# haoningwu3639/StoryGen

Measured on AMD Instinct MI355X. Metric: UNet denoising steps/sec @512x512, 3 prior-frame ctx, bs=1, higher is better.
Workload: dtype f16; 1 GPU; BASELINE configs[1]: StoryGen denoising loop, 512x512 (64x64x4 latent), R=3 prior frames, CFG batch 3, DDIM, SD-1.5 UNet + attn3 (909M params, synthetic fp16 weights); stage=multi-image-condition, samples_per_gpu=1, parallelism=dp1 (one sample per GPU, final all-gather), hipgraph=True, dedup_identical_reference_samples=True, overlap_ref_pass_of_next_step=True, ref_ahead=1, warmup_run=5, split_graphs=False, stream_priority=False, ref_pass_on_cus=0, ref_pass_eager=False, paired_gemm_launches=True, paired_text_image_attention=False, groupnorm_stats_from_epilogues=True, fp16_block_stream=False

## Files before the change

### storygen_amd/csrc/attention.hip

```cpp
#include "attention_kernel.h"

using namespace sgattn;


static int attn_params(const sg_attn_desc* d, AttnParams& p, const char* who) {
    SG_REQUIRE(d != nullptr, "%s: null descriptor", who);
    SG_REQUIRE(d->q && d->k && d->vt && d->o, "%s: null q/k/vt/o", who);
    SG_REQUIRE(d->B > 0 && d->H > 0 && d->Nq > 0 && d->Nk > 0, "%s: bad shape", who);
    if (d->D != 40 && d->D != 80 && d->D != 160)
        return sg_set_error(SG_EUNSUP, "%s: head dim %d not in {40, 80, 160}", who, d->D);
    SG_REQUIRE(d->kv_batches >= 0 && d->kv_batches <= d->B, "%s: kv_batches must be in [0, B]", who);
    SG_REQUIRE(d->ldq % 8 == 0 && d->ldk % 8 == 0 && d->ldvt % 8 == 0 && d->ldo % 4 == 0, "%s: row strides", who);
    SG_REQUIRE(d->bsq % 8 == 0 && d->bsk % 8 == 0 && d->bsvt % 8 == 0 && d->bso % 4 == 0, "%s: batch strides", who);
    SG_REQUIRE(sg_aligned16(d->q) && sg_aligned16(d->k) && sg_aligned16(d->vt) && sg_aligned16(d->o), "%s: 16-byte alignment", who);
    const int64_t hd = (int64_t)d->H * d->D;
    SG_REQUIRE(d->ldq >= hd && d->ldk >= hd && d->ldo >= hd, "%s: token stride smaller than H*D", who);
    SG_REQUIRE(d->ldvt >= ((d->Nk + 7) & ~7), "%s: ldvt must cover Nk rounded up to 8 keys", who);
    SG_REQUIRE((int64_t)d->D * d->ldvt < (1ll << 31), "%s: VT head slab too large for 32-bit offsets", who);
    p = AttnParams{};
    p.q = reinterpret_cast<const f16*>(d->q); p.ldq = d->ldq; p.bsq = d->bsq;
    p.k = reinterpret_cast<const f16*>(d->k); p.ldk = d->ldk; p.bsk = d->bsk;
    p.vt = reinterpret_cast<const f16*>(d->vt); p.ldvt = d->ldvt; p.bsvt = d->bsvt;
    p.o = reinterpret_cast<f16*>(d->o); p.ldo = d->ldo; p.bso = d->bso;
    p.B = d->B; p.H = d->H; p.Nq = d->Nq; p.Nk = d->Nk;
    p.kv_batches = d->kv_batches > 0 ? d->kv_batches : d->B;
    p.scale_log2 = d->scale * 1.44269504088896340736f;
    if (d->kv2_batches > 0) {
        SG_REQUIRE(d->k2 && d->vt2 && d->Nk2 > 0 && d->kv2_batches <= p.kv_batches, "%s: kv2_batches needs k2, vt2, Nk2 and at most kv_batches rows", who);
        SG_REQUIRE(d->bsk2 % 8 == 0 && d->bsvt2 % 8 == 0 && sg_aligned16(d->k2) && sg_aligned16(d->vt2), "%s: k2 / vt2 strides and alignment", who);
        SG_REQUIRE(d->ldvt >= ((d->Nk2 + 7) & ~7), "%s: ldvt must cover Nk2 rounded up to 8 keys", who);
        p.k2 = reinterpret_cast<const f16*>(d->k2); p.bsk2 = d->bsk2;
        p.vt2 = reinterpret_cast<const f16*>(d->vt2); p.bsvt2 = d->bsvt2;
        p.Nk2 = d->Nk2; p.kv2 = d->kv2_batches;
    }
    return SG_OK;
}

static bool attn_big(const sg_attn_desc* d) { return (long)sg_cdiv(d->Nq, 128) * d->H * d->B >= 512; }

static int attn_fwd(const sg_attn_desc* d, float* lse2, sg_stream_t stream) {
    AttnParams p;
    if (int rc = attn_params(d, p, "sg_attn_fwd_f16")) return rc;
    hipStream_t st = (hipStream_t)stream;
    if (lse2) {
        p.lse2 = lse2;
        if (d->D == 40) launch_attn<40, 4, 3, 1, false, true>(p, st);
        else if (d->D == 80) launch_attn<80, 4, 3, 1, false, true>(p, st);
        else launch_attn<160, 4, 3, 1, false, true>(p, st);
        SG_CHECK_LAUNCH("sg_attn_fwd_lse_f16");
        return SG_OK;
    }
    const bool big = attn_big(d);
    const SgOptions& opt = sg_options();
    const int sub2 = opt.attn_sub2, prio = opt.attn_prio;
    if (d->D == 40) {
        if (big && sub2 && d->Nk >= 256) launch_attn<40, 4, 2, 2>(p, st);
        else if (big && prio) launch_attn<40, 4, 3, 1, true>(p, st);
        else if (big && opt.attn_d40_general) launch_attn<40, 4, 3, 1, false, false, false, true>(p, st);
        else if (big && opt.attn_lean) launch_attn<40, 4, 3, 1, false, false, true>(p, st);
        else if (big) launch_attn<40, 4, 3>(p, st);
        else launch_attn<40, 2, 2>(p, st);
    }
    else if (d->D == 80) {
        const int v80 = opt.attn_d80;
        if (v80 == 1 || (v80 == 0 && big)) launch_attn<80, 4, 3>(p, st);
        else if (v80 == 2) launch_attn<80, 2, 3>(p, st);
        else launch_attn<80, 2, 2>(p, st);
    }
    else {
        const int v160 = opt.attn_d160;
        if (v160 == 4 && d->Nq <= 256 && d->Nk > KVBLK && (long)sg_cdiv(d->Nq, 32) * d->H * d->B <= 256) launch_attn_ksplit<160, 4>(p, st);
        else if (v160 == 1) launch_attn<160, 2, 3>(p, st);
        else if (v160 == 2) launch_attn<160, 4, 2>(p, st);
        else if (v160 == 3 || v160 == 4) launch_attn<160, 4, 3>(p, st);
        else launch_attn<160, 2, 2>(p, st);
    }
    SG_CHECK_LAUNCH("sg_attn_fwd_f16");
    return SG_OK;
}

extern "C" int sg_attn_fwd_f16(const sg_attn_desc* d, sg_stream_t stream) { return attn_fwd(d, nullptr, stream); }

extern "C" int sg_attn_fwd_pair_f16(const sg_attn_desc* d0, const sg_attn_desc* d1, sg_stream_t stream) {
    AttnParams p0, p1;
    if (int rc = attn_params(d0, p0, "sg_attn_fwd_pair_f16[0]")) return rc;
    if (int rc = attn_params(d1, p1, "sg_attn_fwd_pair_f16[1]")) return rc;
    const SgOptions& opt = sg_options();
    const bool same = d0->D == d1->D && d0->B == d1->B && d0->H == d1->H && d0->Nq == d1->Nq;
    const bool defaults = !opt.attn_sub2 && !opt.attn_prio && opt.attn_d80 == 1 && opt.attn_d160 >= 3;
    if (!same || !defaults) {
        if (int rc = attn_fwd(d0, nullptr, stream)) return rc;
        return attn_fwd(d1, nullptr, stream);
    }
    const AttnParams& a = p0.Nk >= p1.Nk ? p0 : p1;
    const AttnParams& b = p0.Nk >= p1.Nk ? p1 : p0;
    hipStream_t st = (hipStream_t)stream;
    if (d0->D == 40) {
        if (attn_big(d0)) launch_attn_pair<40, 4, 3>(a, b, st);
        else launch_attn_pair<40, 2, 2>(a, b, st);
    } else if (d0->D == 80) launch_attn_pair<80, 4, 3>(a, b, st);
    else launch_attn_pair<160, 4, 3>(a, b, st);
    SG_CHECK_LAUNCH("sg_attn_fwd_pair_f16");
    return SG_OK;
}

extern "C" int sg_attn_fwd_lse_f16(const sg_attn_desc* d, float* lse2, sg_stream_t stream) {
    SG_REQUIRE(lse2 != nullptr, "sg_attn_fwd_lse_f16: null lse2");
    return attn_fwd(d, lse2, stream);
}
```

### storygen_amd/csrc/attention_kernel.h

```cpp
#pragma once
#include "common.h"
#include <stdlib.h>

namespace sgattn {


constexpr int KVBLK = 64;
constexpr float RESCALE_THR = 6.0f;

struct AttnParams {
    const f16* q; long ldq, bsq;
    const f16* k; long ldk, bsk;
    const f16* vt; long ldvt, bsvt;
    f16* o; long ldo, bso;
    int B, H, Nq, Nk, kv_batches, nqb;
    const f16* k2; long bsk2; const f16* vt2; long bsvt2; int Nk2, kv2;
    float scale_log2;
    float* lse2;
};

__device__ __forceinline__ void glds16(const f16* g, char* lds_wave_base) {
    __builtin_amdgcn_global_load_lds((const __attribute__((address_space(1))) void*)g,
                                     (__attribute__((address_space(3))) void*)lds_wave_base, 16, 0, 0);
}
template <int N>
__device__ __forceinline__ void wait_vmcnt() {
    asm volatile("s_waitcnt vmcnt(%0)" ::"n"(N) : "memory");
}

template <int D>
__device__ __forceinline__ int kswz(int row) {
    return D == 40 ? 0 : (D == 80 ? ((row >> 3) & 1) : ((row >> 2) & 3));
}

constexpr int F40_KPAD = 2688;
constexpr int F40_ONES = 128;

template <int D, int S, int SUB>
constexpr int attn_smem_bytes() {
    return D == 40 ? F40_KPAD + S * SUB * (KVBLK * D * 2 + D * 128 + F40_ONES) : S * SUB * (KVBLK * D * 2 + D * 128) + (D % 16 == 0 ? 0 : 16);
}

#ifdef SG_ATTN_RT_STAGE
constexpr bool UNROLL_STAGES = false;
#else
constexpr bool UNROLL_STAGES = true;
#endif

template <int D, int NW, int S, int SUB, bool PRIO, bool LSE, bool LEAN = false, bool GENERAL = false, bool KSPLIT = false>
__device__ __forceinline__ void attn_fwd_body(const AttnParams& p, char* smem, const int block, const int nblocks) {
    constexpr bool F40 = D == 40 && !GENERAL;
    constexpr int DC = D / 8;
    constexpr int NDK = (D + 15) / 16;
    constexpr int DT = (D + 31) / 32;
    constexpr int KROW = D * 2;
    constexpr int K_BYTES = KVBLK * KROW;
    constexpr int V_BYTES = D * 128;
    constexpr int K_SEG = K_BYTES / 1024, V_SEG = V_BYTES / 1024, NSEG = K_SEG + V_SEG;
    constexpr int TSTAGE = K_BYTES + V_BYTES + (F40 ? F40_ONES : 0);
    constexpr int STAGE = SUB * TSTAGE;
    constexpr int RING0 = F40 ? F40_KPAD : 0;
    constexpr int MAXL = (NSEG + NW - 1) / NW;
    constexpr int REM = NSEG % NW;
    static_assert(KSPLIT ? (S == 1 && SUB == NW && !LSE && !(D == 40 && !GENERAL)) : (S == 2 || S == 3), "2 or 3 stages; key split: one stage of NW tiles");
    static_assert(KSPLIT || SUB == 1 || S == 2, "multi-tile stages use the 2-stage ring (plain vmcnt(0) waits)");
    static_assert(!KSPLIT || NW * (8 + DT * 64) * 64 <= S * SUB * (KVBLK * D * 2 + D * 128), "the merge images of the waves fit the dead ring");
    static_assert((S - 1) * MAXL < 64, "vmcnt is a 6-bit counter");
    static_assert(RING0 + S * STAGE + (F40 || D % 16 == 0 ? 0 : 16) <= attn_smem_bytes<D, S, SUB>(), "LDS size");
    static_assert(!F40 || (32 * KROW + 16 <= F40_KPAD && F40_KPAD % 128 == 0), "K pad constants of both 32-key blocks");

    const int t = threadIdx.x, lane = t & 63, l31 = lane & 31, hi = lane >> 5;
    const int wave = __builtin_amdgcn_readfirstlane(t >> 6);
    const int work = xcd_remap(block, nblocks);
    const int bh = work / p.nqb, qb = work - bh * p.nqb;
    const int h = bh / p.B, b = bh - h * p.B;
    const int kvb = b < p.kv_batches ? b : b - (p.B - p.kv_batches);
    const bool short_row = kvb < p.kv2;
    const int Nk = short_row ? p.Nk2 : p.Nk;
    const int q0 = KSPLIT ? qb * 32 : (qb * NW + wave) * 32;
    const f16* Q = p.q + (long)b * p.bsq + (long)h * D;
    const f16* K = (short_row ? p.k2 + (long)kvb * p.bsk2 : p.k + (long)(kvb - p.kv2) * p.bsk) + (long)h * D;
    const f16* VT = (short_row ? p.vt2 + (long)kvb * p.bsvt2 : p.vt + (long)(kvb - p.kv2) * p.bsvt) + (long)h * D * p.ldvt;
    const int nkp8 = (Nk + 7) & ~7;

    if constexpr (F40) {
// ... 274 lines not shown
            f16x8 vn[VPRE ? 1 : DT];
            if constexpr (!VPRE) {
                if (ks + 1 < 4) {
#pragma unroll
                    for (int i = 0; i < DT; ++i) {
                        const int d = min(i * 32 + l31, DLAST);
                        vn[i] = *reinterpret_cast<const f16x8*>(sV + d * 128 + ((((ks + 1) * 2 + hi) ^ ((d >> 1) & 7)) << 4));
                    }
                }
                __builtin_amdgcn_sched_barrier(0);
            }
            if constexpr (PRIO) __builtin_amdgcn_s_setprio(1);
#pragma unroll
            for (int i = 0; i < DT; ++i)
                oacc[i] = __builtin_amdgcn_mfma_f32_32x32x16_f16(vf[VPRE ? ks : 0][i], pf, oacc[i], 0, 0, 0);
            if constexpr (PRIO) __builtin_amdgcn_s_setprio(0);
            if constexpr (!VPRE) {
                if (ks + 1 < 4) {
#pragma unroll
                    for (int i = 0; i < DT; ++i) vf[0][i] = vn[i];
                }
            }
        }
        }
      }
        }
        if (!UNR && ++rt_stage == S) rt_stage = 0;
    }
    }

    float l_tot;
    if constexpr (F40) l_tot = oacc[DT - 1][4];
    else l_tot = l_run + __shfl_xor(l_run, 32, 64);
    if constexpr (KSPLIT) {
        constexpr int IMG = (8 + DT * 64) * 64;
        __builtin_amdgcn_s_barrier();
        if (wave > 0) {
            float* img = reinterpret_cast<float*>(smem + (wave - 1) * IMG);
            img[lane] = m_run;
            img[64 + lane] = l_tot;
#pragma unroll
            for (int i = 0; i < DT; ++i)
#pragma unroll
                for (int r = 0; r < 16; ++r) img[128 + (i * 16 + r) * 64 + lane] = oacc[i][r];
        }
        asm volatile("s_waitcnt lgkmcnt(0)" ::: "memory");
        __builtin_amdgcn_s_barrier();
        if (wave > 0) return;
#pragma unroll
        for (int w = 1; w < NW; ++w) {
            const float* img = reinterpret_cast<const float*>(smem + (w - 1) * IMG);
            const float m_o = img[lane], l_o = img[64 + lane];
            const float m_new = fmaxf(m_run, m_o);
            const float fa = __builtin_amdgcn_exp2f(m_run - m_new), fb = __builtin_amdgcn_exp2f(m_o - m_new);
            l_tot = l_tot * fa + l_o * fb;
            m_run = m_new;
#pragma unroll
            for (int i = 0; i < DT; ++i)
#pragma unroll
                for (int r = 0; r < 16; ++r) oacc[i][r] = oacc[i][r] * fa + img[128 + (i * 16 + r) * 64 + lane] * fb;
        }
    }
    const float inv = 1.0f / l_tot;
    const int qi = q0 + l31;
    if constexpr (LSE) {
        if (hi == 0 && qi < p.Nq) p.lse2[((long)b * p.H + h) * p.Nq + qi] = m_run + __log2f(l_tot);
    }
    if (qi < p.Nq) {
        f16* O = p.o + (long)b * p.bso + (long)qi * p.ldo + (long)h * D;
#pragma unroll
        for (int i = 0; i < DT; ++i)
#pragma unroll
            for (int g = 0; g < 4; ++g) {
                const int d0 = i * 32 + 8 * g + 4 * hi;
                if (d0 < D) {
                    f16x4 w = {(f16)(oacc[i][4 * g + 0] * inv), (f16)(oacc[i][4 * g + 1] * inv),
                               (f16)(oacc[i][4 * g + 2] * inv), (f16)(oacc[i][4 * g + 3] * inv)};
                    *reinterpret_cast<f16x4*>(O + d0) = w;
                }
            }
    }
}

template <int D, int NW, int S, int SUB = 1, bool PRIO = false, bool LSE = false, bool LEAN = false, bool GENERAL = false>
__global__ __launch_bounds__(64 * NW) void attn_fwd_kernel(const AttnParams p) {
    __shared__ __attribute__((aligned(16))) char smem[attn_smem_bytes<D, S, SUB>()];
    attn_fwd_body<D, NW, S, SUB, PRIO, LSE, LEAN, GENERAL>(p, smem, (int)blockIdx.x, (int)gridDim.x);
}

template <int D, int NW>
__global__ __launch_bounds__(64 * NW) void attn_fwd_ksplit_kernel(const AttnParams p) {
    __shared__ __attribute__((aligned(16))) char smem[attn_smem_bytes<D, 1, NW>()];
    attn_fwd_body<D, NW, 1, NW, false, false, false, false, true>(p, smem, (int)blockIdx.x, (int)gridDim.x);
}

template <int D, int NW>
void launch_attn_ksplit(const AttnParams& p0, hipStream_t st) {
    AttnParams p = p0;
    p.nqb = sg_cdiv(p.Nq, 32);
    hipLaunchKernelGGL((attn_fwd_ksplit_kernel<D, NW>), dim3(p.nqb * p.H * p.B), dim3(64 * NW), 0, st, p);
}

template <int D, int NW, int S>
__global__ __launch_bounds__(64 * NW) void attn_fwd_pair_kernel(const AttnParams a, const AttnParams b, const int na) {
    __shared__ __attribute__((aligned(16))) char smem[attn_smem_bytes<D, S, 1>()];
    if ((int)blockIdx.x < na) attn_fwd_body<D, NW, S, 1, false, false>(a, smem, (int)blockIdx.x, na);
    else attn_fwd_body<D, NW, S, 1, false, false>(b, smem, (int)blockIdx.x - na, (int)gridDim.x - na);
}

template <int D, int NW, int S, int SUB = 1, bool PRIO = false, bool LSE = false, bool LEAN = false, bool GENERAL = false>
void launch_attn(const AttnParams& p0, hipStream_t st) {
    AttnParams p = p0;
    p.nqb = sg_cdiv(p.Nq, 32 * NW);
    hipLaunchKernelGGL((attn_fwd_kernel<D, NW, S, SUB, PRIO, LSE, LEAN, GENERAL>), dim3(p.nqb * p.H * p.B), dim3(64 * NW), 0, st, p);
}

template <int D, int NW, int S>
void launch_attn_pair(const AttnParams& a0, const AttnParams& b0, hipStream_t st) {
    AttnParams a = a0, b = b0;
    a.nqb = sg_cdiv(a.Nq, 32 * NW); b.nqb = sg_cdiv(b.Nq, 32 * NW);
    const int na = a.nqb * a.H * a.B, nb = b.nqb * b.H * b.B;
    hipLaunchKernelGGL((attn_fwd_pair_kernel<D, NW, S>), dim3(na + nb), dim3(64 * NW), 0, st, a, b, na);
}


}
```

### storygen_amd/csrc/common.h

```cpp
#pragma once
#include <hip/hip_runtime.h>
#include <stdint.h>
#include <stdio.h>
#include <stdarg.h>

#include "../../include/storygen_hip.h"

typedef _Float16 f16;
typedef f16 f16x2 __attribute__((ext_vector_type(2)));
typedef f16 f16x4 __attribute__((ext_vector_type(4)));
typedef f16 f16x8 __attribute__((ext_vector_type(8)));
typedef float f32x4 __attribute__((ext_vector_type(4)));
typedef float f32x16 __attribute__((ext_vector_type(16)));

int sg_set_error(int code, const char* fmt, ...);

#define SG_REQUIRE(cond, ...)                                   \
    do {                                                        \
        if (!(cond)) return sg_set_error(SG_EINVAL, __VA_ARGS__); \
    } while (0)

#define SG_CHECK_LAUNCH(name)                                                                  \
    do {                                                                                       \
        hipError_t e__ = hipGetLastError();                                                    \
        if (e__ != hipSuccess) return sg_set_error(SG_ELAUNCH, "%s: %s", name, hipGetErrorString(e__)); \
    } while (0)

static inline bool sg_aligned16(const void* p) { return (reinterpret_cast<uintptr_t>(p) & 15u) == 0; }
static inline int sg_cdiv(long a, long b) { return (int)((a + b - 1) / b); }

struct SgOptions {
    int tile_m = 0, tile_n = 0;
    int no_pipe = 0, no_split = 0;
    int no_nmajor = 0;
    int pipe_stages = 3;
    int lat_tiles = 640;
    int lat_min_kt = 8, lat_max_kt = 64;
    int lat_stages = 4;
    int lat_mask = 62;
    int big_m = 0, big_bm = 0, big_bn = 0;
    int fat_m = 0;
    int lat_wide = 0, lat_wide_m = 256;
    int attn_sub2 = 0, attn_prio = 0, attn_d80 = 1, attn_d160 = 4 , attn_lean = 0;
    int attn_d40_general = 0;
    int gn_no_fused = 0, gn_wide = 1;
    int gn_fused_nt = 1024;
    int gn_chunks = 0;
    int ff_variant = 3;
    long gn_fused_max = -1;
};
SgOptions& sg_options();

__device__ __forceinline__ uint4 ldg16(const void* p) { return *reinterpret_cast<const uint4*>(p); }
__device__ __forceinline__ void stg16(void* p, uint4 v) { *reinterpret_cast<uint4*>(p) = v; }

union H8 {
    uint4 u;
    f16x8 v;
    f16 h[8];
};

__device__ __forceinline__ void load8f(const void* base, long off, bool f32, float (&v)[8]) {
    if (f32) {
        const float* q = reinterpret_cast<const float*>(base) + off;
        const float4 a = *reinterpret_cast<const float4*>(q), b = *reinterpret_cast<const float4*>(q + 4);
        v[0] = a.x; v[1] = a.y; v[2] = a.z; v[3] = a.w; v[4] = b.x; v[5] = b.y; v[6] = b.z; v[7] = b.w;
    } else {
        H8 h; h.u = ldg16(reinterpret_cast<const f16*>(base) + off);
#pragma unroll
        for (int j = 0; j < 8; ++j) v[j] = (float)h.h[j];
    }
}
__device__ __forceinline__ void store8h(f16* p, const float (&v)[8]) {
    H8 o;
#pragma unroll
    for (int j = 0; j < 8; ++j) o.h[j] = (f16)v[j];
    stg16(p, o.u);
}

__device__ __forceinline__ float silu_f(float x) { return x / (1.0f + __expf(-x)); }
__device__ __forceinline__ float gelu_erf_f(float x) {
    const float ax = fabsf(x);
    const float t = __builtin_amdgcn_rcpf(fmaf(ax, 0.3275911f * 0.70710678118654752440f, 1.0f));
    const float zs = ax * 0.84932180028801904272f;
    const float e = __builtin_amdgcn_exp2f(-zs * zs);
    float q = fmaf(1.061405429f, t, -1.453152027f);
    q = fmaf(q, t, 1.421413741f);
    q = fmaf(q, t, -0.284496736f);
    q = fmaf(q, t, 0.254829592f);
    q *= t;
    return 0.5f * fmaf(ax, fmaf(-q, e, 1.0f), x);
}

__device__ __forceinline__ float wave_sum(float v) {
#pragma unroll
    for (int o = 32; o > 0; o >>= 1) v += __shfl_xor(v, o, 64);
    return v;
}

__device__ __forceinline__ int xcd_remap(int bid, int nblocks) {
    const int q = nblocks >> 3, r = nblocks & 7;
    const int xcd = bid & 7, local = bid >> 3;
    const int base = (xcd < r) ? xcd * (q + 1) : r * (q + 1) + (xcd - r) * q;
    return base + local;
}
```

### storygen_amd/csrc/misc.hip

```cpp
#include "common.h"
#include <string.h>

static thread_local char g_err[512] = "";

SgOptions& sg_options() {
    static SgOptions o;
    return o;
}

extern "C" int sg_debug_set_option(const char* name, int64_t value) {
    if (!name) return sg_set_error(SG_EINVAL, "sg_debug_set_option: null name");
    SgOptions& o = sg_options();
    struct Entry { const char* n; int* p; };
    const Entry table[] = {{"tile_m", &o.tile_m}, {"tile_n", &o.tile_n}, {"no_pipe", &o.no_pipe}, {"no_split", &o.no_split},
                           {"no_nmajor", &o.no_nmajor}, {"attn_sub2", &o.attn_sub2}, {"attn_prio", &o.attn_prio},
                           {"attn_d80", &o.attn_d80}, {"attn_d160", &o.attn_d160}, {"gn_no_fused", &o.gn_no_fused},
                           {"gn_wide", &o.gn_wide}, {"attn_lean", &o.attn_lean}, {"attn_d40_general", &o.attn_d40_general},
                           {"gn_fused_nt", &o.gn_fused_nt}, {"pipe_stages", &o.pipe_stages}, {"ff_variant", &o.ff_variant},
                           {"gn_chunks", &o.gn_chunks}, {"lat_tiles", &o.lat_tiles}, {"lat_min_kt", &o.lat_min_kt},
                           {"lat_max_kt", &o.lat_max_kt}, {"lat_stages", &o.lat_stages}, {"lat_wide", &o.lat_wide}, {"lat_mask", &o.lat_mask}, {"lat_wide_m", &o.lat_wide_m}, {"fat_m", &o.fat_m}, {"big_m", &o.big_m}, {"big_bm", &o.big_bm}, {"big_bn", &o.big_bn}};
    for (const Entry& e : table)
        if (strcmp(e.n, name) == 0) {
            *e.p = (int)value;
            return SG_OK;
        }
    if (strcmp(name, "gn_fused_max") == 0) {
        o.gn_fused_max = (long)value;
        return SG_OK;
    }
    if (strcmp(name, "reset") == 0) {
        o = SgOptions{};
        return SG_OK;
    }
    return sg_set_error(SG_EINVAL, "sg_debug_set_option: unknown option '%s'", name);
}

int sg_set_error(int code, const char* fmt, ...) {
    va_list ap;
    va_start(ap, fmt);
    vsnprintf(g_err, sizeof(g_err), fmt, ap);
    va_end(ap);
    return code;
}

extern "C" int sg_version(void) { return 1; }
extern "C" const char* sg_last_error(void) { return g_err; }

extern "C" int sg_device_arch(void) {
    int dev = 0;
    hipDeviceProp_t prop;
    if (hipGetDevice(&dev) != hipSuccess || hipGetDeviceProperties(&prop, dev) != hipSuccess)
        return sg_set_error(SG_ELAUNCH, "sg_device_arch: no HIP device");
    const char* name = prop.gcnArchName;
    if (strncmp(name, "gfx", 3) != 0) return sg_set_error(SG_EARCH, "sg_device_arch: unexpected arch '%s'", name);
    return (int)strtol(name + 3, nullptr, 10);
}

extern "C" int sg_device_cus(void) {
    int dev = 0;
    hipDeviceProp_t prop;
    if (hipGetDevice(&dev) != hipSuccess || hipGetDeviceProperties(&prop, dev) != hipSuccess)
        return sg_set_error(SG_ELAUNCH, "sg_device_cus: no HIP device");
    return prop.multiProcessorCount;
}

namespace {

__global__ void timestep_embed_kernel(const float* t, const float* freqs, float* out, int B, int dim, int flip) {
    const int half = dim / 2;
    const int idx = blockIdx.x * blockDim.x + threadIdx.x;
    if (idx >= B * half) return;
    const int b = idx / half, j = idx - b * half;
    const float e = t[b] * freqs[j];
    const float s = sinf(e), c = cosf(e);
    float* o = out + (long)b * dim;
    if (flip) { o[j] = c; o[half + j] = s; } else { o[j] = s; o[half + j] = c; }
}

template <int MAXB>
__global__ __launch_bounds__(256) void linear_rows_kernel(const float* x, long ldx, const f16* W, long ldw, const f16* bias,
                                                          float* y, long ldy, int B, int N, int K, int act_in, int act_out) {
    const int lane = threadIdx.x & 63, n = blockIdx.x * 4 + (threadIdx.x >> 6);
    if (n >= N) return;
    float acc[MAXB];
#pragma unroll
    for (int b = 0; b < MAXB; ++b) acc[b] = 0.f;
    const f16* wr = W + (long)n * ldw;
    for (int k0 = lane * 8; k0 < K; k0 += 64 * 8) {
        H8 w; w.u = ldg16(wr + k0);
#pragma unroll
        for (int b = 0; b < MAXB; ++b) {
            if (b < B) {
                const float4 x0 = *reinterpret_cast<const float4*>(x + b * ldx + k0);
                const float4 x1 = *reinterpret_cast<const float4*>(x + b * ldx + k0 + 4);
                float xv[8] = {x0.x, x0.y, x0.z, x0.w, x1.x, x1.y, x1.z, x1.w};
#pragma unroll
                for (int j = 0; j < 8; ++j) {
                    const float a = act_in ? silu_f(xv[j]) : xv[j];
                    acc[b] += a * (float)w.h[j];
                }
// ... 337 lines not shown
```

### storygen_amd/ops.py

```python
from __future__ import annotations

import ctypes as C
from typing import Optional

import torch

from . import _lib
from ._lib import AttnDesc, ConvDesc, FfDesc, GemmDesc, GroupNormDesc, check

lib = _lib.load()

EPI_LINEAR = 0
EPI_GEGLU = 1
F_OUT_F32, F_RES1_F32, F_RES2_F32 = 1, 2, 4

TILE_TABLE = {}
TUNE_SINK = None


def _apply_tile(d, tile, split_k, sig, mn):
    if tile is not None:
        d.tile_m, d.tile_n = tile[0], tile[1]
        if len(tile) > 2:
            d.tile_waves = tile[2]
# ... 878 lines not shown
    d = AttnDesc()
    d.q, d.ldq, d.bsq = q.data_ptr(), q.stride(1), q.stride(0)
    d.k, d.ldk, d.bsk = k.data_ptr(), k.stride(1), k.stride(0)
    d.vt, d.ldvt, d.bsvt = vt.data_ptr(), vt.stride(1), vt.stride(0)
    d.o, d.ldo, d.bso = out.data_ptr(), out.stride(1), out.stride(0)
    d.B, d.H, d.Nq, d.Nk, d.D, d.kv_batches, d.scale = B, heads, Nq, Nk, D, (0 if Bk == B else Bk), scale
    return d


def attention_lse(q: torch.Tensor, k: torch.Tensor, vt: torch.Tensor, out: torch.Tensor, lse2: torch.Tensor, heads: int,
                  scale: float, nk: Optional[int] = None) -> torch.Tensor:
    _f32(lse2, "lse2")
    if tuple(lse2.shape) != (q.shape[0], heads, q.shape[1]) or not lse2.is_contiguous():
        raise ValueError("attention_lse: lse2 must be a contiguous [B, H, Nq]")
    d = _attn_desc(q, k, vt, out, heads, scale, nk)
    with _timed(f"attention_d{d.D}", 4.0 * d.B * d.H * d.Nq * d.Nk * d.D, f"B{d.B} H{d.H} Nq{d.Nq} Nk{d.Nk} lse"):
        check(lib.sg_attn_fwd_lse_f16(C.byref(d), lse2.data_ptr(), _stream()), "sg_attn_fwd_lse_f16")
    return out


def attention_bwd_prep(o: torch.Tensor, dout: torch.Tensor, lse2: torch.Tensor, ld2: torch.Tensor, heads: int) -> torch.Tensor:
    _f16(o, "o"), _f16(dout, "dout"), _f32(lse2, "lse2"), _f32(ld2, "ld2")
    B, Nq, Cq = o.shape
    if tuple(ld2.shape) != (B, heads, Nq, 2) or not ld2.is_contiguous() or not lse2.is_contiguous():
        raise ValueError("attention_bwd_prep: ld2 must be a contiguous [B, H, Nq, 2], lse2 a contiguous [B, H, Nq]")
    check(lib.sg_attn_bwd_prep_f32(o.data_ptr(), o.stride(1), o.stride(0), dout.data_ptr(), dout.stride(1), dout.stride(0),
                                   lse2.data_ptr(), ld2.data_ptr(), B, heads, Nq, Cq // heads, _stream()), "sg_attn_bwd_prep_f32")
    return ld2


def _attn_bwd_desc(q, k, v, dout, ld2, heads, scale):
    from ._lib import AttnBwdDesc
    for n, t in (("q", q), ("k", k), ("v", v), ("dout", dout)):
        _f16(t, n)
        if t.dim() != 3 or t.stride(2) != 1:
            raise ValueError(f"attention_bwd: {n} must be [B, N, H*D] with a contiguous last dimension")
    _f32(ld2, "ld2")
    B, Nq, Cq = q.shape
    d = AttnBwdDesc()
    d.q, d.ldq, d.bsq = q.data_ptr(), q.stride(1), q.stride(0)
    d.k, d.ldk, d.bsk = k.data_ptr(), k.stride(1), k.stride(0)
    d.v, d.ldv, d.bsv = v.data_ptr(), v.stride(1), v.stride(0)
    d.dout, d.lddo, d.bsdo = dout.data_ptr(), dout.stride(1), dout.stride(0)
    d.ld2 = ld2.data_ptr()
    d.B, d.H, d.Nq, d.Nk, d.D, d.scale = B, heads, Nq, k.shape[1], Cq // heads, scale
    return d


def attention_bwd_dq(q: torch.Tensor, k: torch.Tensor, kt: torch.Tensor, v: torch.Tensor, dout: torch.Tensor, ld2: torch.Tensor,
                     dq: torch.Tensor, heads: int, scale: float) -> torch.Tensor:
    d = _attn_bwd_desc(q, k, v, dout, ld2, heads, scale)
    _f16(kt, "kt"), _f16(dq, "dq")
    d.kt, d.ldkt, d.bskt = kt.data_ptr(), kt.stride(1), kt.stride(0)
    d.dq, d.lddq, d.bsdq = dq.data_ptr(), dq.stride(1), dq.stride(0)
    with _timed("attention_bwd", 6.0 * d.B * d.H * d.Nq * d.Nk * d.D, f"dq B{d.B} H{d.H} Nq{d.Nq} Nk{d.Nk} D{d.D}"):
        check(lib.sg_attn_bwd_dq_f16(C.byref(d), _stream()), "sg_attn_bwd_dq_f16")
    return dq


def attention_bwd_dkv(q: torch.Tensor, qt: torch.Tensor, k: torch.Tensor, v: torch.Tensor, dout: torch.Tensor, dot: torch.Tensor,
                      ld2: torch.Tensor, dkt: torch.Tensor, dvt: torch.Tensor, heads: int, scale: float):
    d = _attn_bwd_desc(q, k, v, dout, ld2, heads, scale)
    for n, t in (("qt", qt), ("dot", dot), ("dkt", dkt), ("dvt", dvt)):
        _f16(t, n)
    d.qt, d.ldqt, d.bsqt = qt.data_ptr(), qt.stride(1), qt.stride(0)
    d.dot, d.lddot, d.bsdot = dot.data_ptr(), dot.stride(1), dot.stride(0)
    d.dkt, d.lddkt, d.bsdkt = dkt.data_ptr(), dkt.stride(1), dkt.stride(0)
    d.dvt, d.lddvt, d.bsdvt = dvt.data_ptr(), dvt.stride(1), dvt.stride(0)
    with _timed("attention_bwd", 8.0 * d.B * d.H * d.Nq * d.Nk * d.D, f"dkv B{d.B} H{d.H} Nq{d.Nq} Nk{d.Nk} D{d.D}"):
        check(lib.sg_attn_bwd_dkv_f16(C.byref(d), _stream()), "sg_attn_bwd_dkv_f16")
    return dkt, dvt


def debug_set_tile(bm: int = 0, bn: int = 0, no_pipe: bool = False) -> None:
    check(lib.sg_debug_set_tile(bm, bn, int(no_pipe)), "sg_debug_set_tile")


def debug_set_option(name: str, value: int) -> None:
    check(lib.sg_debug_set_option(name.encode(), int(value)), "sg_debug_set_option")


_ENV_OPTIONS = {"SG_NO_NMAJOR": "no_nmajor", "SG_NO_PIPE": "no_pipe", "SG_NO_SPLIT": "no_split",
                "SG_ATTN_SUB2": "attn_sub2", "SG_ATTN_PRIO": "attn_prio", "SG_ATTN_D80": "attn_d80", "SG_ATTN_D160": "attn_d160",
                "SG_FF_VARIANT": "ff_variant", "SG_PIPE_STAGES": "pipe_stages", "SG_GN_FUSED_NT": "gn_fused_nt", "SG_GN_CHUNKS": "gn_chunks", "SG_ATTN_LEAN": "attn_lean", "SG_ATTN_D40_GENERAL": "attn_d40_general", "SG_NO_GN_FUSED": "gn_no_fused", "SG_GN_WIDE": "gn_wide", "SG_GN_FUSED_MAX": "gn_fused_max",
                "SG_LAT_TILES": "lat_tiles", "SG_LAT_MIN_KT": "lat_min_kt", "SG_LAT_MAX_KT": "lat_max_kt", "SG_LAT_STAGES": "lat_stages", "SG_LAT_WIDE": "lat_wide", "SG_LAT_MASK": "lat_mask", "SG_LAT_WIDE_M": "lat_wide_m", "SG_FAT_M": "fat_m", "SG_BIG_M": "big_m", "SG_BIG_BM": "big_bm", "SG_BIG_BN": "big_bn"}


def apply_env_options() -> dict:
    import os
    done = {}
    for var, name in _ENV_OPTIONS.items():
        if os.environ.get(var, "") != "":
            debug_set_option(name, int(os.environ[var]))
            done[name] = int(os.environ[var])
    if os.environ.get("SG_TILE"):
        bm, bn = (int(v) for v in os.environ["SG_TILE"].split(","))
        debug_set_option("tile_m", bm), debug_set_option("tile_n", bn)
        done["tile"] = (bm, bn)
    return done


def debug_mfma_f8(a_bytes: torch.Tensor, b_bytes: torch.Tensor, scale_a: int = 127, scale_b: int = 127) -> torch.Tensor:
    if a_bytes.dtype != torch.uint8 or tuple(a_bytes.shape) != (64, 32) or not a_bytes.is_cuda or not a_bytes.is_contiguous():
        raise TypeError("debug_mfma_f8: a must be a contiguous CUDA uint8 [64, 32]")
    if b_bytes.dtype != torch.uint8 or tuple(b_bytes.shape) != (64, 32) or not b_bytes.is_cuda or not b_bytes.is_contiguous():
        raise TypeError("debug_mfma_f8: b must be a contiguous CUDA uint8 [64, 32]")
    out = torch.empty(64, 16, dtype=torch.float32, device=a_bytes.device)
    check(lib.sg_debug_mfma_f8_32x32x64(a_bytes.data_ptr(), b_bytes.data_ptr(), out.data_ptr(), scale_a, scale_b, _stream()),
          "sg_debug_mfma_f8_32x32x64")
    return out


def debug_mfma(a: torch.Tensor, b: torch.Tensor) -> torch.Tensor:
    out = torch.empty(64, 16, dtype=torch.float32, device=a.device)
    check(lib.sg_debug_mfma_32x32x16(a.data_ptr(), b.data_ptr(), out.data_ptr(), _stream()), "sg_debug_mfma_32x32x16")
    return out
```

Measured before the change: 78.03 denoising steps/s.

## Add specialized head-dim-40 attention kernel with precomputed load offsets and compile-time stages

Adds a dedicated D=40 flash-attention kernel and makes it the default for single and paired launches; the old generic path stays behind an option. It precomputes per-wave global-to-LDS offsets and splits the K/V^T load segments across waves, with waves 0 and 1 loading the extra segment. The main loop is unrolled over compile-time ring stages, and full tiles skip masking. It also folds the running max into the Q fragment so the MFMA subtracts it, and sets waves_per_eu(3). The aim is to cut address arithmetic, branching and masking overhead in the D=40 attention at 64x64 resolution, at the cost of a large new specialized code path that carries precision and correctness risk.

```diff
diff --git a/storygen_amd/csrc/attention.hip b/storygen_amd/csrc/attention.hip
--- a/storygen_amd/csrc/attention.hip
+++ b/storygen_amd/csrc/attention.hip
@@ -58,8 +58,9 @@
         else if (big && prio) launch_attn<40, 4, 3, 1, true>(p, st);
         else if (big && opt.attn_d40_general) launch_attn<40, 4, 3, 1, false, false, false, true>(p, st);
         else if (big && opt.attn_lean) launch_attn<40, 4, 3, 1, false, false, true>(p, st);
-        else if (big) launch_attn<40, 4, 3>(p, st);
-        else launch_attn<40, 2, 2>(p, st);
+        else if (opt.attn_d40_loop == 1) big ? launch_attn<40, 4, 3>(p, st) : launch_attn<40, 2, 2>(p, st);
+        else if (big) launch_attn_d40<4, 3>(p, st);
+        else launch_attn_d40<2, 2>(p, st);
     }
     else if (d->D == 80) {
         const int v80 = opt.attn_d80;
@@ -87,7 +88,8 @@
     if (int rc = attn_params(d1, p1, "sg_attn_fwd_pair_f16[1]")) return rc;
     const SgOptions& opt = sg_options();
     const bool same = d0->D == d1->D && d0->B == d1->B && d0->H == d1->H && d0->Nq == d1->Nq;
-    const bool defaults = !opt.attn_sub2 && !opt.attn_prio && opt.attn_d80 == 1 && opt.attn_d160 >= 3;
+    const bool defaults = !opt.attn_sub2 && !opt.attn_prio && opt.attn_d80 == 1 && opt.attn_d160 >= 3 &&
+                          !(d0->D == 40 && opt.attn_d40_loop == 1);
     if (!same || !defaults) {
         if (int rc = attn_fwd(d0, nullptr, stream)) return rc;
         return attn_fwd(d1, nullptr, stream);
@@ -96,8 +98,8 @@
     const AttnParams& b = p0.Nk >= p1.Nk ? p1 : p0;
     hipStream_t st = (hipStream_t)stream;
     if (d0->D == 40) {
-        if (attn_big(d0)) launch_attn_pair<40, 4, 3>(a, b, st);
-        else launch_attn_pair<40, 2, 2>(a, b, st);
+        if (attn_big(d0)) launch_attn_d40_pair<4, 3>(a, b, st);
+        else launch_attn_d40_pair<2, 2>(a, b, st);
     } else if (d0->D == 80) launch_attn_pair<80, 4, 3>(a, b, st);
     else launch_attn_pair<160, 4, 3>(a, b, st);
     SG_CHECK_LAUNCH("sg_attn_fwd_pair_f16");
diff --git a/storygen_amd/csrc/attention_kernel.h b/storygen_amd/csrc/attention_kernel.h
--- a/storygen_amd/csrc/attention_kernel.h
+++ b/storygen_amd/csrc/attention_kernel.h
@@ -1,6 +1,7 @@
 #pragma once
 #include "common.h"
 #include <stdlib.h>
+#include <type_traits>
 
 namespace sgattn {
 
@@ -441,6 +442,312 @@
     }
 }
 
+template <int NW, int S>
+__device__ __forceinline__ void attn_d40_body(const AttnParams& p, char* smem, const int block, const int nblocks) {
+    constexpr int D = 40, DC = D / 8, NDK = 3, DT = 2, KROW = D * 2;
+    constexpr int K_BYTES = KVBLK * KROW, V_BYTES = D * 128;
+    constexpr int K_SEG = K_BYTES / 1024, V_SEG = V_BYTES / 1024;
+    constexpr int TSTAGE = K_BYTES + V_BYTES + F40_ONES, RING0 = F40_KPAD;
+    constexpr int NPAIR = (K_SEG - 1) / NW;
+    static_assert((NW == 2 || NW == 4) && (S == 2 || S == 3), "2 or 4 waves, 2 or 3 stages");
+    static_assert(K_SEG == 5 && V_SEG == 5 && NPAIR * NW == 4, "4 segments of K and of V^T over the waves + one of each for waves 0 and 1");
+    static_assert(RING0 + S * TSTAGE <= attn_smem_bytes<D, S, 1>(), "LDS size");
+
+    const int t = threadIdx.x, lane = t & 63, l31 = lane & 31, hi = lane >> 5;
+    const int wave = __builtin_amdgcn_readfirstlane(t >> 6);
+    const int work = xcd_remap(block, nblocks);
+    const int bh = work / p.nqb, qb = work - bh * p.nqb;
+    const int h = bh / p.B, b = bh - h * p.B;
+    const int kvb = b < p.kv_batches ? b : b - (p.B - p.kv_batches);
+    const bool short_row = kvb < p.kv2;
+    const int Nk = short_row ? p.Nk2 : p.Nk;
+    const int q0 = (qb * NW + wave) * 32;
+    const f16* Q = p.q + (long)b * p.bsq + (long)h * D;
+    const f16* K = (short_row ? p.k2 + (long)kvb * p.bsk2 : p.k + (long)(kvb - p.kv2) * p.bsk) + (long)h * D;
+    const f16* VT = (short_row ? p.vt2 + (long)kvb * p.bsvt2 : p.vt + (long)(kvb - p.kv2) * p.bsvt) + (long)h * D * p.ldvt;
+    const int nkp8 = (Nk + 7) & ~7;
+    const int ntiles = (Nk + KVBLK - 1) / KVBLK, nfull = Nk / KVBLK;
+    const int ldk = (int)p.ldk, ldvt = (int)p.ldvt;
+
+    if (t < 8) {
+        const unsigned v = (t & 3) == 0 ? 0x3C003C00u : 0u;
+        *reinterpret_cast<unsigned*>(smem + ((t >> 2) ? 32 * KROW : 0) + 4 * (t & 3)) = v;
+    }
+    for (int i = t; i < S * (F40_ONES / 4); i += 64 * NW) {
+        const int img = i / (F40_ONES / 4), w = i - img * (F40_ONES / 4);
+        *reinterpret_cast<unsigned*>(smem + RING0 + img * TSTAGE + K_BYTES + V_BYTES + 4 * w) = 0x3C003C00u;
+    }
+    asm volatile("s_waitcnt lgkmcnt(0)" ::: "memory");
+
+    auto kcoord = [&](int seg, int& row, int& col) __attribute__((always_inline)) {
+        const int s = seg * 64 + lane;
+        row = s / DC;
+        col = (s - row * DC) * 8;
+    };
+    auto vcoord = [&](int seg, int& row, int& col) __attribute__((always_inline)) {
+        const int s = seg * 64 + lane;
+        const int d = s >> 3, cs = s & 7;
+        row = d * ldvt;
+        col = (cs ^ ((d >> 1) & 7)) * 8;
+    };
+    unsigned koff[NPAIR], voff[NPAIR], xoff;
+    {
+        int row, col;
+#pragma unroll
+        for (int j = 0; j < NPAIR; ++j) {
+            kcoord(j * NW + wave, row, col);
+            koff[j] = (unsigned)(row * ldk + col);
+            vcoord(j * NW + wave, row, col);
+            voff[j] = (unsigned)(row + col);
+        }
+        kcoord(K_SEG - 1, row, col);
+        const unsigned xk = (unsigned)(row * ldk + col);
+        vcoord(V_SEG - 1, row, col);
+        xoff = wave == 0 ? xk : (unsigned)(row + col);
+    }
+    const int xdst = wave == 0 ? (K_SEG - 1) * 1024 : K_BYTES + (V_SEG - 1) * 1024;
+
+    auto issue_full = [&](auto has3, const f16* Kt, const f16* Vt, const f16* Xt, char* base) __attribute__((always_inline)) {
+#pragma unroll
+        for (int j = 0; j < NPAIR; ++j) glds16(Kt + koff[j], base + (j * NW + wave) * 1024);
+#pragma unroll
+        for (int j = 0; j < NPAIR; ++j) glds16(Vt + voff[j], base + K_BYTES + (j * NW + wave) * 1024);
+        if constexpr (decltype(has3)::value) glds16(Xt + xoff, base + xdst);
+    };
+    auto issue_any = [&](auto has3, int tile, char* base) __attribute__((always_inline)) {
+        const int key0 = tile * KVBLK;
+        if (key0 + KVBLK <= Nk) {
+            const f16* Kt = K + (long)key0 * ldk;
+            const f16* Vt = VT + key0;
+            issue_full(has3, Kt, Vt, wave == 0 ? Kt : Vt, base);
+        } else {
+            auto ktail = [&](int seg) __attribute__((always_inline)) {
+                int row, col;
+                kcoord(seg, row, col);
+                glds16(K + (long)min(key0 + row, Nk - 1) * ldk + col, base + seg * 1024);
+            };
+            auto vtail = [&](int seg) __attribute__((always_inline)) {
+                int row, col;
+                vcoord(seg, row, col);
+                glds16(VT + row + min(key0 + col, nkp8 - 8), base + K_BYTES + seg * 1024);
+            };
+#pragma unroll
+            for (int j = 0; j < NPAIR; ++j) ktail(j * NW + wave);
+#pragma unroll
+            for (int j = 0; j < NPAIR; ++j) vtail(j * NW + wave);
+            if constexpr (decltype(has3)::value) {
+                if (wave == 0) ktail(K_SEG - 1);
+                else vtail(V_SEG - 1);
+            }
+        }
+    };
+
+    f16x8 qf[NDK];
+    {
+        const int qi = min(q0 + l31, p.Nq - 1);
+#pragma unroll
+        for (int s = 0; s < NDK; ++s) {
+            const int d0 = s * 16 + hi * 8;
+            H8 x; x.u = make_uint4(0, 0, 0, 0);
+            if (d0 < D) x.u = ldg16(Q + (long)qi * p.ldq + d0);
+#pragma unroll
+            for (int j = 0; j < 8; ++j) x.h[j] = (f16)((float)x.h[j] * p.scale_log2);
+            qf[s] = x.v;
+        }
+    }
+    __builtin_amdgcn_s_waitcnt(0x0F70);
+
+    f32x16 oacc[DT];
+#pragma unroll
+    for (int i = 0; i < DT; ++i)
+#pragma unroll
+        for (int r = 0; r < 16; ++r) oacc[i][r] = 0.f;
+    float m_run = 0.f;
+
+    const int prow = (l31 & ~12) | ((l31 & 4) << 1) | ((l31 & 8) >> 1);
+
+    auto compute = [&](auto first_, auto mask_, auto stage_, const int tile) __attribute__((always_inline)) {
+        constexpr bool FIRST = decltype(first_)::value, MASK = decltype(mask_)::value;
+        constexpr int STG = decltype(stage_)::value;
+        const char* sK = smem + RING0 + STG * TSTAGE;
+        const char* sV = sK + K_BYTES;
+        f32x16 s[2];
+        const f32x16 zero16 = {0.f, 0.f, 0.f, 0.f, 0.f, 0.f, 0.f, 0.f, 0.f, 0.f, 0.f, 0.f, 0.f, 0.f, 0.f, 0.f};
+        f16x8 kf[2][NDK];
+        const char* k01 = sK + prow * KROW + hi * 16;
+        const char* k2 = hi ? smem : sK + prow * KROW + 64;
+#pragma unroll
+        for (int kb = 0; kb < 2; ++kb) {
+            kf[kb][0] = *reinterpret_cast<const f16x8*>(k01 + kb * 32 * KROW);
+            kf[kb][1] = *reinterpret_cast<const f16x8*>(k01 + kb * 32 * KROW + 32);
+            kf[kb][2] = *reinterpret_cast<const f16x8*>(k2 + kb * 32 * KROW);
+        }
+        __builtin_amdgcn_sched_barrier(0);
+#pragma unroll
+        for (int kb = 0; kb < 2; ++kb)
+#pragma unroll
+            for (int st = 0; st < NDK; ++st)
+                s[kb] = __builtin_amdgcn_mfma_f32_32x32x16_f16(kf[kb][st], qf[st], st == 0 ? zero16 : s[kb], 0, 0, 0);
+        f16x8 vf[4][DT];
+#pragma unroll
+        for (int ks = 0; ks < 4; ++ks)
+#pragma unroll
+            for (int i = 0; i < DT; ++i) {
+                const int d = min(i * 32 + l31, D);
+                vf[ks][i] = *reinterpret_cast<const f16x8*>(sV + d * 128 + (((ks * 2 + hi) ^ ((d >> 1) & 7)) << 4));
+            }
+        if constexpr (MASK) {
+            if ((tile + 1) * KVBLK > Nk) {
+#pragma unroll
+                for (int kb = 0; kb < 2; ++kb)
+#pragma unroll
+                    for (int r = 0; r < 16; ++r) {
+                        const int key = tile * KVBLK + kb * 32 + 16 * (r >> 3) + 8 * hi + (r & 7);
+                        if (key >= Nk) s[kb][r] = -INFINITY;
+                    }
+            }
+        }
+        float mx = s[0][0];
+#pragma unroll
+        for (int kb = 0; kb < 2; ++kb)
+#pragma unroll
+            for (int r = 0; r < 16; ++r) mx = fmaxf(mx, s[kb][r]);
+        mx = fmaxf(mx, __shfl_xor(mx, 32, 64));
+        if (FIRST || __builtin_amdgcn_ballot_w64(mx > RESCALE_THR) != 0) {
+            float m_new = m_run + (FIRST ? mx : fmaxf(mx, 0.f));
+            m_new = fminf(fmaxf(m_new, -60000.f), 60000.f);
+            const f16 mh = (f16)m_new;
+            const f16 ml = (f16)(m_new - (float)mh);
+            m_new = (float)mh + (float)ml;
+            const float delta = m_new - m_run;
+            if constexpr (!FIRST) {
+                const float alpha = __builtin_amdgcn_exp2f(-delta);
+#pragma unroll
+                for (int i = 0; i < DT; ++i)
+#pragma unroll
+                    for (int r = 0; r < 16; ++r) oacc[i][r] *= alpha;
+            }
+#pragma unroll
+            for (int kb = 0; kb < 2; ++kb)
+#pragma unroll
+                for (int r = 0; r < 16; ++r) s[kb][r] -= delta;
+            m_run = m_new;
+            if (hi) { qf[NDK - 1][0] = -mh; qf[NDK - 1][1] = -ml; }
+        }
+#pragma unroll
+        for (int kb = 0; kb < 2; ++kb)
+#pragma unroll
+            for (int r = 0; r < 16; ++r) s[kb][r] = __builtin_amdgcn_exp2f(s[kb][r]);
+#pragma unroll
+        for (int ks = 0; ks < 4; ++ks) {
+            f16x8 pf;
+#pragma unroll
+            for (int j = 0; j < 8; ++j) pf[j] = (f16)s[ks >> 1][(ks & 1) * 8 + j];
+#pragma unroll
+            for (int i = 0; i < DT; ++i)
+                oacc[i] = __builtin_amdgcn_mfma_f32_32x32x16_f16(vf[ks][i], pf, oacc[i], 0, 0, 0);
+        }
+    };
+
+    char* const ring = smem + RING0;
+    auto run = [&](auto has3) __attribute__((always_inline)) {
+        constexpr int NP = 2 * NPAIR + (decltype(has3)::value ? 1 : 0);
+        static_assert((S - 1) * NP < 64, "vmcnt is a 6-bit counter");
+        using T = std::true_type;
+        using F = std::false_type;
+#pragma unroll
+        for (int s = 0; s < S - 1; ++s)
+            if (s < ntiles) issue_any(has3, s, ring + s * TSTAGE);
+        if (S == 3 && 1 < ntiles) wait_vmcnt<NP>();
+        else wait_vmcnt<0>();
+        __builtin_amdgcn_s_barrier();
+        if (S - 1 < ntiles) issue_any(has3, S - 1, ring + (S - 1) * TSTAGE);
+        compute(T{}, T{}, std::integral_constant<int, 0>{}, 0);
+
+        int tile = 1;
+        const long kstep = (long)KVBLK * ldk;
+        const f16* Kn = K + S * kstep;
+        const f16* Vn = VT + S * KVBLK;
+        const f16* Xn = wave == 0 ? Kn : Vn;
+        const long xstep = wave == 0 ? kstep : (long)KVBLK;
+        for (; tile + 2 * S - 2 < nfull; tile += S) {
+            auto step = [&](auto stage_) __attribute__((always_inline)) {
+                constexpr int STG = decltype(stage_)::value;
+                wait_vmcnt<(S == 3 ? NP : 0)>();
+                __builtin_amdgcn_s_barrier();
+                issue_full(has3, Kn, Vn, Xn, ring + ((STG + S - 1) % S) * TSTAGE);
+                Kn += kstep; Vn += KVBLK; Xn += xstep;
+                compute(F{}, F{}, stage_, 0);
+            };
+            step(std::integral_constant<int, 1 % S>{});
+            step(std::integral_constant<int, 2 % S>{});
+            if constexpr (S == 3) step(std::integral_constant<int, 0>{});
+        }
+        for (; tile < ntiles; tile += S) {
+            auto step = [&](auto stage_, const int tl) __attribute__((always_inline)) {
+                constexpr int STG = decltype(stage_)::value;
+                if (tl < ntiles) {
+                    if (S == 3 && tl + 1 < ntiles) wait_vmcnt<NP>();
+                    else wait_vmcnt<0>();
+                    __builtin_amdgcn_s_barrier();
+                    if (tl + S - 1 < ntiles) issue_any(has3, tl + S - 1, ring + ((STG + S - 1) % S) * TSTAGE);
+                    compute(F{}, T{}, stage_, tl);
+                }
+            };
+            step(std::integral_constant<int, 1 % S>{}, tile);
+            step(std::integral_constant<int, 2 % S>{}, tile + 1);
+            if constexpr (S == 3) step(std::integral_constant<int, 0>{}, tile + 2);
+        }
+    };
+    if (NW == 4 && wave >= 2) run(std::false_type{});
+    else run(std::true_type{});
+
+    const float inv = 1.0f / oacc[DT - 1][4];
+    const int qi = q0 + l31;
+    if (qi < p.Nq) {
+        f16* O = p.o + (long)b * p.bso + (long)qi * p.ldo + (long)h * D;
+#pragma unroll
+        for (int i = 0; i < DT; ++i)
+#pragma unroll
+            for (int g = 0; g < 4; ++g) {
+                const int d0 = i * 32 + 8 * g + 4 * hi;
+                if (d0 < D) {
+                    f16x4 w = {(f16)(oacc[i][4 * g + 0] * inv), (f16)(oacc[i][4 * g + 1] * inv),
+                               (f16)(oacc[i][4 * g + 2] * inv), (f16)(oacc[i][4 * g + 3] * inv)};
+                    *reinterpret_cast<f16x4*>(O + d0) = w;
+                }
+            }
+    }
+}
+
+template <int NW, int S>
+__global__ __launch_bounds__(64 * NW) __attribute__((amdgpu_waves_per_eu(3))) void attn_d40_kernel(const AttnParams p) {
+    __shared__ __attribute__((aligned(16))) char smem[attn_smem_bytes<40, S, 1>()];
+    attn_d40_body<NW, S>(p, smem, (int)blockIdx.x, (int)gridDim.x);
+}
+
+template <int NW, int S>
+__global__ __launch_bounds__(64 * NW) __attribute__((amdgpu_waves_per_eu(3))) void attn_d40_pair_kernel(const AttnParams a, const AttnParams b, const int na) {
+    __shared__ __attribute__((aligned(16))) char smem[attn_smem_bytes<40, S, 1>()];
+    if ((int)blockIdx.x < na) attn_d40_body<NW, S>(a, smem, (int)blockIdx.x, na);
+    else attn_d40_body<NW, S>(b, smem, (int)blockIdx.x - na, (int)gridDim.x - na);
+}
+
+template <int NW, int S>
+void launch_attn_d40(const AttnParams& p0, hipStream_t st) {
+    AttnParams p = p0;
+    p.nqb = sg_cdiv(p.Nq, 32 * NW);
+    hipLaunchKernelGGL((attn_d40_kernel<NW, S>), dim3(p.nqb * p.H * p.B), dim3(64 * NW), 0, st, p);
+}
+
+template <int NW, int S>
+void launch_attn_d40_pair(const AttnParams& a0, const AttnParams& b0, hipStream_t st) {
+    AttnParams a = a0, b = b0;
+    a.nqb = sg_cdiv(a.Nq, 32 * NW); b.nqb = sg_cdiv(b.Nq, 32 * NW);
+    const int na = a.nqb * a.H * a.B, nb = b.nqb * b.H * b.B;
+    hipLaunchKernelGGL((attn_d40_pair_kernel<NW, S>), dim3(na + nb), dim3(64 * NW), 0, st, a, b, na);
+}
+
 template <int D, int NW, int S, int SUB = 1, bool PRIO = false, bool LSE = false, bool LEAN = false, bool GENERAL = false>
 __global__ __launch_bounds__(64 * NW) void attn_fwd_kernel(const AttnParams p) {
     __shared__ __attribute__((aligned(16))) char smem[attn_smem_bytes<D, S, SUB>()];
diff --git a/storygen_amd/csrc/common.h b/storygen_amd/csrc/common.h
--- a/storygen_amd/csrc/common.h
+++ b/storygen_amd/csrc/common.h
@@ -43,6 +43,7 @@
     int lat_wide = 0, lat_wide_m = 256;
     int attn_sub2 = 0, attn_prio = 0, attn_d80 = 1, attn_d160 = 4 , attn_lean = 0;
     int attn_d40_general = 0;
+    int attn_d40_loop = 0;
     int gn_no_fused = 0, gn_wide = 1;
     int gn_fused_nt = 1024;
     int gn_chunks = 0;
diff --git a/storygen_amd/csrc/misc.hip b/storygen_amd/csrc/misc.hip
--- a/storygen_amd/csrc/misc.hip
+++ b/storygen_amd/csrc/misc.hip
@@ -15,7 +15,7 @@
     const Entry table[] = {{"tile_m", &o.tile_m}, {"tile_n", &o.tile_n}, {"no_pipe", &o.no_pipe}, {"no_split", &o.no_split},
                            {"no_nmajor", &o.no_nmajor}, {"attn_sub2", &o.attn_sub2}, {"attn_prio", &o.attn_prio},
                            {"attn_d80", &o.attn_d80}, {"attn_d160", &o.attn_d160}, {"gn_no_fused", &o.gn_no_fused},
-                           {"gn_wide", &o.gn_wide}, {"attn_lean", &o.attn_lean}, {"attn_d40_general", &o.attn_d40_general},
+                           {"gn_wide", &o.gn_wide}, {"attn_lean", &o.attn_lean}, {"attn_d40_general", &o.attn_d40_general}, {"attn_d40_loop", &o.attn_d40_loop},
                            {"gn_fused_nt", &o.gn_fused_nt}, {"pipe_stages", &o.pipe_stages}, {"ff_variant", &o.ff_variant},
                            {"gn_chunks", &o.gn_chunks}, {"lat_tiles", &o.lat_tiles}, {"lat_min_kt", &o.lat_min_kt},
                            {"lat_max_kt", &o.lat_max_kt}, {"lat_stages", &o.lat_stages}, {"lat_wide", &o.lat_wide}, {"lat_mask", &o.lat_mask}, {"lat_wide_m", &o.lat_wide_m}, {"fat_m", &o.fat_m}, {"big_m", &o.big_m}, {"big_bm", &o.big_bm}, {"big_bn", &o.big_bn}};
diff --git a/storygen_amd/ops.py b/storygen_amd/ops.py
--- a/storygen_amd/ops.py
+++ b/storygen_amd/ops.py
@@ -984,7 +984,7 @@
 
 _ENV_OPTIONS = {"SG_NO_NMAJOR": "no_nmajor", "SG_NO_PIPE": "no_pipe", "SG_NO_SPLIT": "no_split",
                 "SG_ATTN_SUB2": "attn_sub2", "SG_ATTN_PRIO": "attn_prio", "SG_ATTN_D80": "attn_d80", "SG_ATTN_D160": "attn_d160",
-                "SG_FF_VARIANT": "ff_variant", "SG_PIPE_STAGES": "pipe_stages", "SG_GN_FUSED_NT": "gn_fused_nt", "SG_GN_CHUNKS": "gn_chunks", "SG_ATTN_LEAN": "attn_lean", "SG_ATTN_D40_GENERAL": "attn_d40_general", "SG_NO_GN_FUSED": "gn_no_fused", "SG_GN_WIDE": "gn_wide", "SG_GN_FUSED_MAX": "gn_fused_max",
+                "SG_FF_VARIANT": "ff_variant", "SG_PIPE_STAGES": "pipe_stages", "SG_GN_FUSED_NT": "gn_fused_nt", "SG_GN_CHUNKS": "gn_chunks", "SG_ATTN_LEAN": "attn_lean", "SG_ATTN_D40_GENERAL": "attn_d40_general", "SG_ATTN_D40_LOOP": "attn_d40_loop","SG_NO_GN_FUSED": "gn_no_fused", "SG_GN_WIDE": "gn_wide", "SG_GN_FUSED_MAX": "gn_fused_max",
                 "SG_LAT_TILES": "lat_tiles", "SG_LAT_MIN_KT": "lat_min_kt", "SG_LAT_MAX_KT": "lat_max_kt", "SG_LAT_STAGES": "lat_stages", "SG_LAT_WIDE": "lat_wide", "SG_LAT_MASK": "lat_mask", "SG_LAT_WIDE_M": "lat_wide_m", "SG_FAT_M": "fat_m", "SG_BIG_M": "big_m", "SG_BIG_BM": "big_bm", "SG_BIG_BN": "big_bn"}
 
 
```

Measured after the change: 78.84 denoising steps/s (median of 6 runs). 1.01x the previous value.
